# lefarov/Ape-X-DQN

Measured on AMD Instinct MI355X. Metric: learner grad-steps/sec at batch 512, 84x84x4 dueling DQN, higher is better.
Workload: dtype fp32; 1 GPU; model=dueling NatureCNN (reference DuellingDQN, conv1=64), 4x84x84, A=4, global_batch=512, seq_len=1, parallelism=dp1, batch_scope=global, per_rank_rows=512, replay_per_gpu=100000, learner=fused/hip, hip_graphs=True

## Files before the change

### apex_dqn_amd/learner/fused_learner.py

```python
from __future__ import annotations

from typing import Any, Dict, Optional

import torch

from ..config import ApexConfig
from ..models.dueling import DuellingDQN
from ..models.flat_params import (FlatLayout, flat_to_reference_state, nature_segments,
                                  reference_state_to_flat)
from ..ops.fused_ops import HipBackend, TorchBackend, split_into
from ..ops.switches import SW
from ..utils.checkpoint import (adopt_obs_scale, layout_segments, load_checkpoint, pack_flat_state,
                                save_checkpoint, unpack_flat_state, checkpoint_network)
from .dp_step import DataParallelStep, Streams
from .is_norm import IsNormMixin


def _enable_sharding(replay, comm, rt, mcap: int = 0) -> None:
    if not replay.sharded:
        seed0 = comm.broadcast_int(int(rt.seed)) if hasattr(comm, "broadcast_int") else int(rt.seed)
        replay.enable_sharding(comm.rank, comm.world_size, shard_seed=(seed0 << 20) ^ 0x5EED,
                               group=comm.group, mcap=mcap)
    replay.shard_mcap = int(mcap)
    if not rt.use_is_weights:
# ... 248 lines not shown
        if self._branched or self._dp:
            return
        nrm = (self.norm_part, 0) if self._fuse_norm else None
        self._fc_slots = ops.fc_head_wgrad(self.dH, self.y3[:B], self.G["wfc"], self.G["bfc"], self.h,
                                           self.dhead, self.G, prio, norm=nrm,
                                           **self._lo(dh_lo=self.dH_lo, x_lo=sp and self.y3_lo[:B],
                                                      Hon_lo=self.h_lo))
        if self._comm_bf16:
            cut = self.layout.offsets["wfc"]
            self.gcomm[cut:].copy_(self.g32[cut:])
        self._mark("fc_wgrad")

    def _sample(self) -> None:
        self.replay.sample(self.B, out=self.S, nxt2=self.slots[2 * self.B:])
        self._sample_ver = self.replay.version

    def _seg2(self, after_first=None) -> None:
        if self._branched:
            assert after_first is None
            return self._seg2_branched()
        B, rt, ops, G, Pb, Pl = self.B, self.rt, self.ops, self.G, self.Pb, self.Pl
        sp = self.split
        jobs = []
        ops.fc_dgrad(self.dH, self.y3[:B], Pb["wfc"], self.dY3,
                     **self._lo(dh_lo=self.dH_lo, w_lo=sp and Pl["wfc"], dx_lo=self.dY3_lo))
        if after_first is not None:
            after_first()
        ops.conv_wgrad(self.dY3, self.y2[:B], 3, 1, G["w3"], G["b3"], jobs=jobs,
                       **self._lo(dy_lo=self.dY3_lo, x_lo=sp and self.y2_lo[:B]))
        ops.conv_dgrad(self.dY3, Pb["w3"], 1, self.y2[:B], self.dY2,
                       **self._lo(dy_lo=self.dY3_lo, w_lo=sp and Pl["w3"], dx_lo=self.dY2_lo))
        ops.conv_wgrad(self.dY2, self.y1[:B], 4, 2, G["w2"], G["b2"], jobs=jobs,
                       **self._lo(dy_lo=self.dY2_lo, x_lo=sp and self.y1_lo[:B]))
        ops.conv_dgrad(self.dY2, Pb["w2"], 2, self.y1[:B], self.dY1,
                       **self._lo(dy_lo=self.dY2_lo, w_lo=sp and Pl["w2"], dx_lo=self.dY1_lo))
        jobs1 = []
        ops.conv1_wgrad_ring(self.dY1, self.replay.frames, self.slots[:B], self.frames, rt.obs_scale, G["w1"],
                             G["b1"], jobs=jobs1, **self._lo(dy_lo=self.dY1_lo))
        fuse = self._fuse_norm
        n1 = ops.finalize_grads(jobs, self.g_head_region if fuse else None,
                                dict(part=self.norm_part, slot0=self._fc_slots) if fuse else None)
        n2 = ops.finalize_grads(jobs1, None, dict(part=self.norm_part, slot0=n1) if fuse else None)
        self._npart = n2 if fuse else 0
        if self._comm_bf16:
            cut = self.layout.offsets["wfc"]
            self.gcomm[:cut].copy_(self.g32[:cut])
        self._mark("conv_backward")

    _marks = None

    def _mark(self, name: str) -> None:
        if self._marks is not None:
            ev = torch.cuda.Event(enable_timing=True)
            ev.record()
            self._marks.append((name, ev))

    def profile_step(self) -> Dict[str, float]:
        if self.device.type != "cuda":
            return {}
        start = torch.cuda.Event(enable_timing=True)
        start.record()
        self._marks = []
        try:
            if self._dp:
                self._dp_body()
            else:
                self._step_body()
        finally:
            marks, self._marks = self._marks, None
        torch.cuda.synchronize(self.device)
        out, prev = {}, start
# ... 17 lines not shown
                      **({"frag_out": self._frag_out} if (self._frag_out is not None and nxt is not None) else {}),
                      **({"segs": segs} if segs is not None else {}),
                      **({"norm_prefix": norm_prefix} if norm_prefix is not None else {}))
        if self._presample:
            self._sample_ver = self.replay.version
        self._mark("optimizer")

    def _seg2_branched(self) -> None:
        B, rt, ops, G, Pb, Pl, S = self.B, self.rt, self.ops, self.G, self.Pb, self.Pl, self.S
        sp = self.split
        main, side = torch.cuda.current_stream(self.device), self._wg_stream
        jobs = []
        prio = (self.replay, S["idx"], S["gen"], self.td_abs)
        nrm = (self.norm_part, 0) if self._fuse_norm else None

        def fc_wgrad():
            self._fc_slots = ops.fc_head_wgrad(self.dH, self.y3[:B], G["wfc"], G["bfc"], self.h, self.dhead, G,
                                               prio, norm=nrm,
                                               **self._lo(dh_lo=self.dH_lo, x_lo=sp and self.y3_lo[:B],
                                                          Hon_lo=self.h_lo))

        fc_main = SW.fc_wgrad_main == "on" or (SW.fc_wgrad_main == "auto" and sp and B >= 256)
        if not fc_main:
            ev = torch.cuda.Event()
            ev.record(main)
        ops.fc_dgrad(self.dH, self.y3[:B], Pb["wfc"], self.dY3,
                     **self._lo(dh_lo=self.dH_lo, w_lo=sp and Pl["wfc"], dx_lo=self.dY3_lo))
        if fc_main:
            fc_wgrad()
        else:
            side.wait_event(ev)
            with torch.cuda.stream(side):
                fc_wgrad()
        self._conv32_branched(main, side, jobs)
        fuse = self._fuse_norm
        jobs1 = []
        ops.conv1_wgrad_ring(self.dY1, self.replay.frames, self.slots[:B], self.frames, rt.obs_scale, G["w1"],
                             G["b1"], jobs=jobs1, **self._lo(dy_lo=self.dY1_lo))
        with torch.cuda.stream(side):
            n_side = ops.finalize_grads(jobs, self.g_head_region if fuse else None,
                                        dict(part=self.norm_part, slot0=self._fc_slots) if fuse else None)
        n_main = ops.finalize_grads(jobs1, None, dict(part=self.norm_part, slot0=n_side) if fuse else None)
        main.wait_stream(side)
        self._npart = n_main
        self._mark("conv_backward")

    def _conv2_wgrad(self, jobs) -> None:
        B, sp = self.B, self.split
        self.ops.conv_wgrad(self.dY2, self.y1[:B], 4, 2, self.G["w2"], self.G["b2"], jobs=jobs,
                            **self._lo(dy_lo=self.dY2_lo, x_lo=sp and self.y1_lo[:B]))

    def _conv3_wgrad(self, jobs) -> None:
        B, sp = self.B, self.split
        self.ops.conv_wgrad(self.dY3, self.y2[:B], 3, 1, self.G["w3"], self.G["b3"], jobs=jobs,
                            **self._lo(dy_lo=self.dY3_lo, x_lo=sp and self.y2_lo[:B]))

    def _conv32_branched(self, main, side, jobs, wgrad2: bool = True) -> None:
        B, ops, G, Pb, Pl, sp = self.B, self.ops, self.G, self.Pb, self.Pl, self.split
        ev3 = torch.cuda.Event()
        ev3.record(main)
        ops.conv_dgrad(self.dY3, Pb["w3"], 1, self.y2[:B], self.dY2,
                       **self._lo(dy_lo=self.dY3_lo, w_lo=sp and Pl["w3"], dx_lo=self.dY2_lo))
        side.wait_event(ev3)
        with torch.cuda.stream(side):
            self._conv3_wgrad(jobs)
        ev2 = torch.cuda.Event()
        ev2.record(main)
        ops.conv_dgrad(self.dY2, Pb["w2"], 2, self.y1[:B], self.dY1,
                       **self._lo(dy_lo=self.dY2_lo, w_lo=sp and Pl["w2"], dx_lo=self.dY1_lo))
        side.wait_event(ev2)
        if wgrad2:
            with torch.cuda.stream(side):
                self._conv2_wgrad(jobs)

    def _step_body(self) -> None:
        self._seg1()
        self._seg2()
        self._seg3()

    def _body(self) -> None:
        if self._dp:
            self._dp_body()
        else:
            self._step_body()
        if not self._defer_params:
            self._wait_params()

    _step_hook = None

    graph_fallback = None
    _inject_capture_failure = False

    def _graphs_enabled(self) -> bool:
        return (bool(self.rt.use_graphs) and self.device.type == "cuda" and (not self._dp or self._dp_graphs)
                and self.graph_fallback is None)

    def step(self) -> None:
        graphs = self._graphs_enabled()
        if graphs and self._graphs is None:
            self.prepare_graphs(multi=False)
            graphs = self._graphs_enabled()
        if graphs and self._presample and self._sample_ver != self.replay.version:
# ... 281 lines not shown
```

### apex_dqn_amd/ops/conv.py

```python
from __future__ import annotations

from typing import Dict, Optional, Tuple


import torch

from . import _lib
from .switches import SW


class Workspace:
    def __init__(self):
        self.bufs: Dict[Tuple, torch.Tensor] = {}

    def get(self, key, numel: int, device, dtype=torch.float32) -> torch.Tensor:
        k = (key, numel, str(device), dtype)
        t = self.bufs.get(k)
        if t is None:
            t = torch.empty(numel, dtype=dtype, device=device)
            self.bufs[k] = t
        return t

    work_queue = False

    def wq(self, key, device, overlapped: bool = True) -> int:
        mode = SW.work_queue
        on = mode == "on" or (mode != "off" and self.work_queue and overlapped)
        return self.get_zeroed(key, 1, device, dtype=torch.int64).data_ptr() if on else 0

    def get_zeroed(self, key, numel: int, device, dtype=torch.int32) -> torch.Tensor:
        k = (key, numel, str(device), dtype)
        t = self.bufs.get(k)
        if t is None:
            t = torch.zeros(numel, dtype=dtype, device=device)
            self.bufs[k] = t
        return t


_DEFAULT_WS = Workspace()

_HINTS: Dict[str, int] = {}


def set_launch_hints(tile: int = 0, order: int = 0) -> None:
    _HINTS["tile"], _HINTS["order"] = int(tile), int(order)


def _conv_desc(**kw) -> "_lib.ConvDesc":
    d = _lib.ConvDesc()
    d.x = kw.get("x")
    d.frame_slots = kw.get("frame_slots")
    d.w = kw["w"]
    d.bias = kw.get("bias")
    d.y = kw["y"]
    d.mask = kw.get("mask")
    d.N, d.H, d.W, d.Cin = kw["N"], kw.get("H", 1), kw.get("W", 1), kw["Cin"]
    d.OH, d.OW, d.Cout = kw.get("OH", 1), kw.get("OW", 1), kw["Cout"]
    d.KH, d.KW = kw.get("KH", 1), kw.get("KW", 1)
    d.stride, d.pad_h, d.pad_w = kw.get("stride", 1), kw.get("pad", 0), kw.get("pad", 0)
    d.mode, d.relu = kw["mode"], int(kw.get("relu", 0))
# ... 391 lines not shown
               "conv_wgrad")


def conv1_wgrad_ring(lib, ws: Workspace, dy: torch.Tensor, ring: torch.Tensor, slots: torch.Tensor,
                     scale: float, dw_out: torch.Tensor, db_out: torch.Tensor, grid: int = 0,
                     jobs: Optional[list] = None, dy_lo: Optional[torch.Tensor] = None) -> None:
    N, OH, OW, Co = dy.shape
    C = slots.shape[1]
    assert (OH, OW, Co) == (20, 20, 64) and slots.dtype == torch.int32 and dy.is_contiguous()
    G = grid if grid > 0 else min(N, 256)
    K = 64 * C
    slab = ws.get(("wg1img", C, G), G * 64 * K, dy.device)
    bslab = ws.get(("wg1imgb", G), G * 64, dy.device)
    zero = ws.get(("zero16",), 64, ring.device, torch.uint8)
    if not getattr(ws, "_zeroed", False):
        zero.zero_()
        ws._zeroed = True
    d = _lib.Conv1WgDesc()
    d.ring, d.slots, d.dy = ring.data_ptr(), slots.data_ptr(), dy.data_ptr()
    d.slab, d.bias_slab, d.zero16 = slab.data_ptr(), bslab.data_ptr(), zero.data_ptr()
    d.N, d.C = N, C
    d.dy_lo = _lib.ptr(dy_lo)
    d.wq = ws.wq(("c1w_wq", N, int(G)), dy.device)
    st = _lib.stream_ptr()
    _lib.check(lib.apex_conv1_wgrad_img(d, G, st), "conv1_wgrad_img")
    if jobs is not None:
        jobs.append(dict(slab=slab, bslab=bslab, out=dw_out, bout=db_out, n=64 * K, nsplit=G, nb=64, s2dC=C, Kc=K,
                         scale=float(scale)))
        return
    _lib.check(lib.apex_slab_reduce(slab.data_ptr(), G, 64 * K, float(scale), dw_out.data_ptr(), bslab.data_ptr(),
                                    64, db_out.data_ptr(), C, K, st), "slab_reduce")


def conv1_wgrad_ring_tiled(lib, ws: Workspace, dy: torch.Tensor, ring: torch.Tensor, slots: torch.Tensor,
                           scale: float, dw_out: torch.Tensor, db_out: torch.Tensor, target_rows: int = 0,
                           jobs: Optional[list] = None, dy_lo: Optional[torch.Tensor] = None) -> None:
    if target_rows <= 0:
        target_rows = 800 if dy_lo is not None else 1024
    N, OH, OW, Co = dy.shape
    C = slots.shape[1]
    Kc = C * 64
    Mred = N * OH * OW
    nsplit, rows = _splits(Mred, target_rows, _WG_TBL // C)
    slab = ws.get(("wg1", Co, Kc), nsplit * Co * Kc, dy.device)
    bslab = ws.get(("wg1b", Co), nsplit * Co, dy.device)
    d = _wg_desc(dy=dy.data_ptr(), x=ring.data_ptr(), frame_slots=slots.data_ptr(), slab=slab.data_ptr(),
                 bias_slab=bslab.data_ptr(), N=N, H=ring.shape[1], W=ring.shape[2], Cin=C, OH=OH, OW=OW,
                 KH=8, KW=8, stride=4, mode=2, Co=Co, Kc=Kc, ldd=Co, rows_per_split=rows, Mred=Mred,
                 dy_lo=_lib.ptr(dy_lo))
    if jobs is not None:
        _lib.check(lib.apex_conv_wgrad(d, None, None, nsplit, 1.0, _lib.stream_ptr()), "conv1_wgrad")
        jobs.append(dict(slab=slab, bslab=bslab, out=dw_out, bout=db_out, n=Co * Kc, nsplit=nsplit, nb=Co, s2dC=C,
                         Kc=Kc, scale=float(scale)))
        return
    _lib.check(lib.apex_conv_wgrad(d, dw_out.data_ptr(), db_out.data_ptr(), nsplit, float(scale),
                                   _lib.stream_ptr()), "conv1_wgrad")


_WG_SHAPES = ((1, 4), (2, 2), (4, 1), (1, 3), (1, 1), (1, 2), (2, 1))


def wgrad_blocks(Co: int, Kc: int, sp: int = 0) -> int:
    kt, ct = Kc // 64, Co // 64
    best, bc = (1, 1), None
    for i, (c, n) in enumerate(_WG_SHAPES):
        if kt % n or ct % c:
# ... 106 lines not shown
```

### apex_dqn_amd/ops/conv_sigs.py

```python
from __future__ import annotations

import ctypes

c_p = ctypes.c_void_p
c_i = ctypes.c_int
c_i64 = ctypes.c_int64
c_f = ctypes.c_float


class Conv2ImgDesc(ctypes.Structure):
    _fields_ = [("x", c_p), ("w", c_p), ("w2", c_p), ("bias", c_p), ("bias2", c_p), ("y", c_p),
                ("N", c_i), ("img_switch", c_i), ("x_lo", c_p), ("w_lo", c_p), ("w2_lo", c_p), ("y_lo", c_p),
                ("wfrag", c_p), ("wfrag_ready", c_i)]


class Conv12Desc(ctypes.Structure):
    _fields_ = [("ring", c_p), ("slots", c_p), ("w1", c_p), ("w1b", c_p), ("b1", c_p), ("b1b", c_p),
                ("w2", c_p), ("w2_lo", c_p), ("w2b", c_p), ("w2b_lo", c_p), ("wfrag", c_p), ("pack_sets", c_i),
                ("b2", c_p), ("b2b", c_p), ("y1", c_p), ("y1_lo", c_p), ("y2", c_p), ("y2_lo", c_p),
                ("w1frag", c_p), ("scratch", c_p), ("N", c_i), ("C", c_i), ("img_switch", c_i), ("copy_n", c_i),
                ("in_scale", ctypes.c_float), ("probe", c_p), ("wq", c_p), ("bf16", c_i), ("probe_split", c_i),
                ("w3", c_p), ("w3_lo", c_p), ("w3b", c_p), ("w3b_lo", c_p), ("b3", c_p), ("b3b", c_p),
                ("y3", c_p), ("y3_lo", c_p), ("w3frag", c_p)]


class Conv2DgradImgDesc(ctypes.Structure):
    _fields_ = [("dy", c_p), ("w", c_p), ("mask", c_p), ("dx", c_p), ("N", c_i), ("dy_lo", c_p), ("w_lo", c_p),
                ("dx_lo", c_p), ("wfrag", c_p), ("wfrag_ready", c_i), ("wq", c_p), ("cls_split", c_i)]


class C2dPackJob(ctypes.Structure):
    _fields_ = [("w", c_p), ("w_lo", c_p), ("out", c_p)]


class Conv3DgradImgDesc(ctypes.Structure):
    _fields_ = [("dy", c_p), ("w", c_p), ("mask", c_p), ("dx", c_p), ("N", c_i)]


def declare(lib: ctypes.CDLL) -> None:
    from ._lib import ConvDesc, WgradDesc
    sigs = {
        "apex_conv2_img_fwd": ([Conv2ImgDesc, c_i, c_p], c_i),
        "apex_conv12_fused_fwd": ([Conv12Desc, c_i, c_p], c_i),
        "apex_conv12_pack": ([Conv12Desc, c_p], c_i),
        "apex_conv2_dgrad_img": ([Conv2DgradImgDesc, c_i, c_p], c_i),
        "apex_conv3_dgrad_img": ([Conv3DgradImgDesc, c_i, c_p], c_i),
        "apex_conv_fwd": ([ConvDesc, c_p], c_i),
        "apex_fc_gemm128": ([ConvDesc, c_p, c_i64, c_i, c_i, c_i, C2dPackJob, c_p], c_i),
        "apex_conv_wgrad": ([WgradDesc, c_p, c_p, c_i, c_f, c_p], c_i),
        "apex_pack_dgrad_weights": ([c_p, c_p, c_p, c_p, c_p, c_p, c_p], c_i),
    }
    for name, (args, res) in sigs.items():
        fn = getattr(lib, name, None)
        if fn is None:
            continue
        fn.argtypes = args
        fn.restype = res
```

### apex_dqn_amd/ops/fused_ops.py

```python
from __future__ import annotations

import ctypes
from typing import Dict, Optional

import torch

from . import _lib
from . import conv as C
from . import reference as R
from .switches import SW


def join(hi: torch.Tensor, lo: Optional[torch.Tensor]) -> torch.Tensor:
    return hi.float() if lo is None else hi.float() + lo.float()


def split_into(v: torch.Tensor, hi: torch.Tensor, lo: Optional[torch.Tensor]) -> None:
    hi.copy_(v.reshape(hi.shape))
    if lo is not None:
        lo.copy_((v.reshape(hi.shape).float() - hi.float()))


class TorchBackend:
    name = "torch"
# ... 171 lines not shown

    def fc_wgrad_split(self, dh, x, dw_out, db_out, jobs, split_rows: int, jnorm, dh_lo=None, x_lo=None,
                       cpb: int = -1) -> int:
        return self.fc_wgrad(dh, x, dw_out, db_out, norm=(jnorm, 0), dh_lo=dh_lo, x_lo=x_lo)

    def fc_head_wgrad(self, dh, x, dw_out, db_out, Hon, dhead, g_head, prio, norm=None, dh_lo=None, x_lo=None,
                      Hon_lo=None) -> int:
        self.head_wgrad(Hon, dhead, g_head, prio=prio, Hon_lo=Hon_lo)
        return self.fc_wgrad(dh, x, dw_out, db_out, norm=norm, dh_lo=dh_lo, x_lo=x_lo) or 0

    def finalize_grads(self, jobs, norm_range=None, norm=None) -> int:
        return 0

    def conv_dgrad(self, dy, w, stride, x_src, dx_out, dy_lo=None, w_lo=None, dx_lo=None):
        if dy_lo is not None:
            dx = R.conv_dgrad(join(dy, dy_lo), join(w, w_lo), tuple(x_src.shape), stride, x_src, torch.float32)
            split_into(dx, dx_out, dx_lo)
            return
        dx_out.copy_(R.conv_dgrad(dy, w, tuple(x_src.shape), stride, x_src, self.dtype))

    def conv_wgrad(self, dy, x, k, stride, dw_out, db_out, jobs=None, dy_lo=None, x_lo=None):
        dw, db = R.conv_wgrad(join(dy, dy_lo), join(x, x_lo), k, stride)
        dw_out.copy_(dw)
        db_out.copy_(db)

    def conv1_wgrad(self, dy, frames, scale, dw_out, db_out, dy_lo=None):
        dw, db = R.conv1_wgrad(join(dy, dy_lo), frames, scale)
        dw_out.copy_(dw)
        db_out.copy_(db)

    def conv1_wgrad_ring(self, dy, ring, slots, frames_buf, scale, dw_out, db_out, jobs=None, dy_lo=None):
        self.conv1_wgrad(dy, frames_buf[:slots.shape[0]], scale, dw_out, db_out, dy_lo=dy_lo)

    def optimizer(self, p32, g32, v, m, pbf, lr, alpha, eps, clip, centered, partials, norm_out, norm_total=None,
                  sample=None, pb_lo=None, wnorm=None, frag_out=None, segs=None, norm_prefix=None):
        self._optimizer(p32, g32, v, m, pbf, lr, alpha, eps, clip, centered, norm_out, pb_lo, wnorm, norm_total,
                        segs, norm_prefix)
        if sample is not None:
            rp, B, out, nxt2 = sample
            rp.sample(B, out=out, nxt2=nxt2)

    def _optimizer(self, p32, g32, v, m, pbf, lr, alpha, eps, clip, centered, norm_out, pb_lo=None, wnorm=None,
                   norm_total=None, segs=None, norm_prefix=None):
        sc = torch.ones((), dtype=torch.float32, device=g32.device)
        if wnorm is not None:
            st, n, stride = wnorm
            mx = st.reshape(-1)[0:n * stride:stride].max().float()
            sc = torch.where(mx > 0, 1.0 / mx.clamp_min(1e-30), sc)
        if norm_total is not None:
            part, npart = norm_total if isinstance(norm_total, tuple) else (norm_total, 1)
            sq = part[:npart].double().sum()
            if norm_prefix is not None:
                sq = sq + norm_prefix.double().pow(2).sum()
        else:
            assert segs is None, "a sharded update needs the clip norm's partials (norm_total)"
            sq = g32.double().pow(2).sum()
        norm = sq.sqrt().float() * sc
        coef = torch.clamp(clip / (norm + 1e-6), max=1.0) if clip > 0 else torch.ones_like(norm)
        for o, n in (segs if segs is not None else [(0, p32.numel())]):
            r = slice(o, o + n)
            g = g32[r] * (coef * sc)
            vr, mr, pr = v[r], m[r], p32[r]
            vr.mul_(alpha).add_((1 - alpha) * g * g)
            if centered:
                mr.mul_(alpha).add_((1 - alpha) * g)
                var = vr - mr * mr
# ... 139 lines not shown
                return r
        return super().fc_head_wgrad(dh, x, dw_out, db_out, Hon, dhead, g_head, prio, norm, dh_lo, x_lo, Hon_lo)

    def finalize_grads(self, jobs, norm_range=None, norm=None) -> int:
        if not jobs and norm is None:
            return 0
        if norm is None:
            C.finalize_grads(self.lib, jobs)
            return 0
        return norm["slot0"] + C.finalize_grads(self.lib, jobs, norm_range, norm["part"], norm["slot0"],
                                                norm.get("total"))

    def conv_dgrad(self, dy, w, stride, x_src, dx_out, dy_lo=None, w_lo=None, dx_lo=None):
        if not self.native_conv:
            return super().conv_dgrad(dy, w, stride, x_src, dx_out, dy_lo, w_lo, dx_lo)
        if stride == 1:
            C.conv3_dgrad(self.lib, dy, w, x_src, dx_out, dy_lo=dy_lo, w_lo=w_lo, out_lo=dx_lo)
        else:
            key = (w.data_ptr(), _lib.ptr(w_lo))
            packed = getattr(self, "_c2d_packed", None) == key
            self._c2d_packed = None
            C.conv2_dgrad(self.lib, dy, w, x_src, dx_out, dy_lo=dy_lo, w_lo=w_lo, out_lo=dx_lo, ws=self.ws,
                          packed=packed)

    def conv_wgrad(self, dy, x, k, stride, dw_out, db_out, jobs=None, dy_lo=None, x_lo=None):
        if not self.native_conv:
            return super().conv_wgrad(dy, x, k, stride, dw_out, db_out, dy_lo=dy_lo, x_lo=x_lo)
        C.conv_wgrad(self.lib, self.ws, dy, x, k, stride, dw_out, db_out, jobs=jobs, dy_lo=dy_lo, x_lo=x_lo)

    def conv1_wgrad_ring(self, dy, ring, slots, frames_buf, scale, dw_out, db_out, jobs=None, dy_lo=None):
        if not self.native_conv:
            return super().conv1_wgrad_ring(dy, ring, slots, frames_buf, scale, dw_out, db_out, dy_lo=dy_lo)
        C.conv1_wgrad_ring(self.lib, self.ws, dy, ring, slots, scale, dw_out, db_out, jobs=jobs, dy_lo=dy_lo)

    @staticmethod
    def _hp(P):
        h = _lib.HeadParams()
        h.wv, h.bv, h.wa, h.ba = (P["wv"].data_ptr(), P["bv"].data_ptr(), P["wa"].data_ptr(),
                                  P["ba"].data_ptr())
        return h

    def head(self, Hon, Htg, Pon, Ptg, act, rew, gam, isw, huber, kappa, grad_scale, td_abs, loss, dH,
             dhead, q_out=None, zero=None, lo=None, isn=None):
        B = act.shape[0]
        A = Pon["wa"].shape[0]
        args = (Hon.data_ptr(), Htg.data_ptr(), self._hp(Pon), self._hp(Ptg), act.data_ptr(), rew.data_ptr(),
                gam.data_ptr(), _lib.ptr(isw), B, A, int(huber), float(kappa), float(grad_scale),
                td_abs.data_ptr(), loss.data_ptr(), _lib.ptr(q_out), dH.data_ptr(), dhead.data_ptr(),
                _lib.ptr(zero), 0 if zero is None else zero.numel(), Pon["wv"].numel())
        hl = _lib.head_lo(*(lo if lo is not None else (None, None, None)))
        hp, pk = _lib.HeadPart(), _lib.C2dPack()
        fp = getattr(self, "_fc_part", None)
        if fp is not None:
            self._fc_part = None
            assert fp["out"].data_ptr() == Hon.data_ptr() and fp["two_b"] == 2 * B
            hp.part, hp.zstride, hp.nz = fp["part"].data_ptr(), int(fp["zstride"]), int(fp["nz"])
            hp.bias_on, hp.bias_tg, hp.two_b = fp["b"].data_ptr(), fp["b2"].data_ptr(), int(fp["two_b"])
            hp.hon, hp.hon_lo = Hon.data_ptr(), _lib.ptr(None if lo is None else lo[0])
            if fp["c2d"] is not None:
                pk.w, pk.w_lo = fp["c2d"][0].data_ptr(), _lib.ptr(fp["c2d"][1])
                pk.out = C.c2d_wfrag_buffer(self.ws, Hon.device).data_ptr()
                self._c2d_packed = (fp["c2d"][0].data_ptr(), _lib.ptr(fp["c2d"][1]))
        isn_s = _lib.IsNorm()
        if isn is not None:
            isn_s.wscale, isn_s.out = _lib.ptr(isn[0]), _lib.ptr(isn[1])
            isn_s.valid_count = _lib.ptr(isn[2]) if len(isn) > 2 else None
# ... 117 lines not shown
```

### apex_dqn_amd/ops/switches.py

```python
from __future__ import annotations

import dataclasses
import os
from dataclasses import dataclass
from typing import Any, Dict


@dataclass
class Switches:
    conv2_img: bool = True
    c2f_pack: bool = True
    conv12_fused: bool = True
    conv123_max_images: int = 1 << 20
    conv12_bf16: bool = True
    conv3_dgrad_img: bool = True
    conv2_dgrad_img: bool = True
    conv2_dgrad_cls_max: int = 256
    opt_frags: bool = True
    fc_epi_in_head: bool = True
    bwd_branches: bool = True
    actor_fc_ksplit: int = 4
    fc_wgrad_main: str = "auto"
    fc_ksplit_max: int = 0
    work_queue: str = "auto"
    wg_rows3: int = 0
    wg_rows2: int = 0
    impala_wg_target: int = 512
    impala_slab_cap: int = 8 << 20
    resblock_r16: int = 14
    impala_pool_wgrad: bool = True
    isplit_bands: str = ""
    dp_fc_shard_branch: bool = False
    dp_branch_one_wait: bool = True
    dp_fc_split_rows: int = -1
    dp_norm_split: bool = True

    @classmethod
    def from_env(cls, spec: str = None) -> "Switches":
        sw = cls()
        spec = os.environ.get("APEX_SWITCHES", "") if spec is None else spec
        for item in spec.split(","):
            item = item.strip()
            if not item:
                continue
            if "=" not in item:
                raise ValueError(f"APEX_SWITCHES item must be name=value, got {item!r}")
            k, v = item.split("=", 1)
            f = {f.name: f for f in dataclasses.fields(cls)}.get(k)
            if f is None:
                raise ValueError(f"unknown kernel switch {k!r}")
# ... 20 lines not shown
```

Baseline: 2705 grad-steps/s (batch 512).

## Fuse conv2 dgrad with conv1 wgrad into one persistent per-image HIP kernel

Adds a persistent kernel that computes conv2's input gradient per image in LDS, applies the ReLU mask, and immediately uses that tile together with DMA-loaded ring frames to accumulate conv1 weight and bias gradients into per-block slabs. The intermediate dY1 no longer needs to be written to and re-read from global memory, and one kernel launch is removed from the backward pass. The kernel uses large LDS and 512 threads with one block per CU, and pipelines the next image's frame and dy loads behind the current image's MFMA work. It is enabled by default on the branched and unbranched backward paths when batch exceeds the class-split threshold, C=4, and the work queue is off. A fallback to the previous two-kernel path is kept.

```diff
diff --git a/apex_dqn_amd/csrc/conv21_bwd_fused.hip b/apex_dqn_amd/csrc/conv21_bwd_fused.hip
--- /dev/null
+++ b/apex_dqn_amd/csrc/conv21_bwd_fused.hip
@@ -0,0 +1,299 @@
+#include "mfma_common.h"
+#include "conv2_wfrag.h"
+
+typedef float f32x16 __attribute__((ext_vector_type(16)));
+
+struct Conv21BwdDesc {
+  const bf16_t* dy;
+  const bf16_t* dy_lo;
+  const bf16_t* w;
+  const bf16_t* w_lo;
+  const bf16_t* mask;
+  uint4* wfrag;
+  int wfrag_ready;
+  const uint8_t* ring;
+  const int32_t* slots;
+  const uint8_t* zero16;
+  float* slab;
+  float* bias_slab;
+  bf16_t* dx;
+  bf16_t* dx_lo;
+  unsigned long long* wq;
+  int N, C;
+};
+
+#define F21_THREADS 512
+#define F21_PLANE 7168
+#define F21_IMG (8 * F21_PLANE)
+#define F21_DYPL (256 * 128)
+#define F21_S2PL (144 * 128)
+#define F21_NCHUNK (4 * 441)
+#define F21_NDMA 28
+#define F21_NDY2 11
+
+__device__ __forceinline__ int f21_c2d_off(int slot, int c) { return (slot << 7) + ((c ^ ((slot >> 1) & 7)) << 4); }
+
+__global__ void __launch_bounds__(256) pack_c2d_wfrag21_kernel(const bf16_t* __restrict__ w,
+                                                               const bf16_t* __restrict__ w_lo,
+                                                               uint32_t* __restrict__ out) {
+  pack_c2d_wfrag_word(blockIdx.x * 256 + threadIdx.x, w, w_lo, out);
+}
+
+__global__ void __launch_bounds__(F21_THREADS, 1) conv21_bwd_fused_kernel(Conv21BwdDesc d) {
+  __shared__ __attribute__((aligned(16))) uint8_t smem[F21_IMG + 2 * F21_DYPL + 2 * F21_S2PL];
+  uint8_t* Pl = smem;
+  uint8_t* Dy = Pl + F21_IMG;
+  uint8_t* S2 = Dy + 2 * F21_DYPL;
+  uint8_t* Sg = S2;
+  const int tid = threadIdx.x, lane = tid & 63;
+  const int wv = __builtin_amdgcn_readfirstlane(tid >> 6);
+  const int cls = wv >> 1, nh = wv & 1, p = cls >> 1, q = cls & 1;
+  const int rr = lane & 31, kg = lane >> 5;
+  const int g = lane >> 4, qq = (lane >> 2) & 3, pcol = lane & 3;
+  const int wc = wv & 1, wk = wv >> 1;
+  const int G = gridDim.x;
+
+  bf16x8 wh[16], wl[16];
+  {
+    const uint4* __restrict__ wf = d.wfrag + ((cls * 2 + nh) * 16) * 64 + lane;
+#pragma unroll
+    for (int s = 0; s < 16; ++s) {
+      wh[s] = __builtin_bit_cast(bf16x8, wf[s * 64]);
+      wl[s] = __builtin_bit_cast(bf16x8, wf[C2D_FRAGS + s * 64]);
+    }
+  }
+  int xoff[4];
+#pragma unroll
+  for (int j = 0; j < 4; ++j)
+    xoff[j] = (2 * j + (pcol >> 1)) * F21_PLANE + (((wk >> 1) * 21 + (wk & 1)) << 4) + ((pcol & 1) << 3);
+
+  auto issue_frames = [&](int img) {
+    int sl[4];
+    sload_slots<4>(d.slots + img * 4, sl);
+    int ln = lane;
+    asm volatile("" : "+v"(ln));
+#pragma unroll
+    for (int i = 0; i < 4; ++i) {
+      const int k = wv * 4 + i;
+      if (k < F21_NDMA) {
+        const int j = 64 * k + ln;
+        const uint8_t* src = d.zero16;
+        if (j < F21_NCHUNK) {
+          const int c = j / 441, blk = j - c * 441;
+          int slot = sl[0];
+#pragma unroll
+          for (int cc = 1; cc < 4; ++cc)
+            if (c == cc) slot = sl[cc];
+          src = d.ring + (int64_t)slot * 7056 + (blk << 4);
+        }
+        const uint32_t off = (uint32_t)(uintptr_t)(__attribute__((address_space(3))) uint8_t*)(Sg + k * 1024);
+        dma16(src, __builtin_amdgcn_readfirstlane(off));
+      }
+    }
+  };
+  auto convert_frames = [&]() {
+    for (int j = tid; j < F21_NCHUNK; j += F21_THREADS) {
+      const uint4 v = *reinterpret_cast<const uint4*>(Sg + j * 16);
+      const int c = j / 441, blk = j - c * 441;
+      *reinterpret_cast<uint4*>(Pl + (2 * c) * F21_PLANE + blk * 16) = u8x8_to_bf16x8(v.x, v.y);
+      *reinterpret_cast<uint4*>(Pl + (2 * c + 1) * F21_PLANE + blk * 16) = u8x8_to_bf16x8(v.z, v.w);
+    }
+  };
+  auto issue_dy2 = [&](int img) {
+    int ln = lane;
+    asm volatile("" : "+v"(ln));
+#pragma unroll
+    for (int i = 0; i < 3; ++i) {
+      const int k = wv + 8 * i;
+      if (k < 2 * F21_NDY2) {
+        const int pln = k / F21_NDY2, kk = k - pln * F21_NDY2, j = 64 * kk + ln;
+        const uint8_t* src = d.zero16;
+        if (j < 81 * 8) src = reinterpret_cast<const uint8_t*>((pln ? d.dy_lo : d.dy) + (int64_t)img * 81 * 64) + j * 16;
+        const uint32_t off =
+            (uint32_t)(uintptr_t)(__attribute__((address_space(3))) uint8_t*)(Dy + pln * F21_DYPL + 160 * 128 + kk * 1024);
+        dma16(src, __builtin_amdgcn_readfirstlane(off));
+      }
+    }
+  };
+  auto store_dy2 = [&]() {
+    for (int k = tid; k < 2 * 144 * 8; k += F21_THREADS) {
+      const int pl = k >= 144 * 8 ? 1 : 0, kk = k - pl * 144 * 8;
+      const int slot = kk >> 3, c = (kk & 7) ^ ((slot >> 1) & 7);
+      const int row = slot / 11, col = slot - row * 11;
+      uint4 v = make_uint4(0, 0, 0, 0);
+      if (row >= 1 && row <= 9 && col >= 1 && col <= 9)
+        v = *reinterpret_cast<const uint4*>(Dy + pl * F21_DYPL + 160 * 128 + (((row - 1) * 9 + col - 1) * 8 + c) * 16);
+      *reinterpret_cast<uint4*>(S2 + k * 16) = v;
+    }
+  };
+
+  f32x4 acc[2][4], accb[2];
+#pragma unroll
+  for (int i = 0; i < 2; ++i) {
+    accb[i] = (f32x4){0.f, 0.f, 0.f, 0.f};
+#pragma unroll
+    for (int j = 0; j < 4; ++j) acc[i][j] = (f32x4){0.f, 0.f, 0.f, 0.f};
+  }
+  const bf16x8 ones = __builtin_bit_cast(bf16x8, make_uint4(0x3f803f80u, 0x3f803f80u, 0x3f803f80u, 0x3f803f80u));
+
+  auto wg_steps = [&](int ks0, int ks1, int lk0) {
+#pragma unroll 1
+    for (int ks = ks0; ks < ks1; ++ks) {
+      const int p0 = min(32 * ks + 8 * g + qq, 399), p1 = min(32 * ks + 8 * g + qq + 4, 399);
+      const int oh0 = p0 / 20, oh1 = p1 / 20;
+      const int b0 = ((oh0 * 21 + p0 - 20 * oh0) << 4), b1 = ((oh1 * 21 + p1 - 20 * oh1) << 4);
+      const int lk = ks - ks0 + lk0;
+      bf16x8 a[2], al[2], b[4];
+#pragma unroll
+      for (int i = 0; i < 2; ++i) {
+        a[i] = tr_frag8(Dy, lk, 16 * (2 * wc + i), lane);
+        al[i] = tr_frag8(Dy + F21_DYPL, lk, 16 * (2 * wc + i), lane);
+      }
+#pragma unroll
+      for (int j = 0; j < 4; ++j) {
+        const lds_s16x4* pa = (const lds_s16x4*)(Pl + b0 + xoff[j]);
+        const lds_s16x4* pb = (const lds_s16x4*)(Pl + b1 + xoff[j]);
+        s16x4 lo = __builtin_amdgcn_ds_read_tr16_b64_v4i16(const_cast<lds_s16x4*>(pa));
+        s16x4 hi = __builtin_amdgcn_ds_read_tr16_b64_v4i16(const_cast<lds_s16x4*>(pb));
+        typedef short s16x8 __attribute__((ext_vector_type(8)));
+        b[j] = __builtin_bit_cast(bf16x8, (s16x8){lo[0], lo[1], lo[2], lo[3], hi[0], hi[1], hi[2], hi[3]});
+      }
+#pragma unroll
+      for (int i = 0; i < 2; ++i)
+#pragma unroll
+        for (int j = 0; j < 4; ++j) {
+          acc[i][j] = __builtin_amdgcn_mfma_f32_16x16x32_bf16(b[j], al[i], acc[i][j], 0, 0, 0);
+          acc[i][j] = __builtin_amdgcn_mfma_f32_16x16x32_bf16(b[j], a[i], acc[i][j], 0, 0, 0);
+        }
+      if (wk == 0) {
+#pragma unroll
+        for (int i = 0; i < 2; ++i) {
+          accb[i] = __builtin_amdgcn_mfma_f32_16x16x32_bf16(ones, al[i], accb[i], 0, 0, 0);
+          accb[i] = __builtin_amdgcn_mfma_f32_16x16x32_bf16(ones, a[i], accb[i], 0, 0, 0);
+        }
+      }
+    }
+  };
+
+  int img = blockIdx.x;
+  if (img < d.N) {
+    issue_dy2(img);
+    issue_frames(img);
+  }
+  for (; img < d.N; img += G) {
+    asm volatile("s_waitcnt vmcnt(0)" ::: "memory");
+    __syncthreads();
+    convert_frames();
+    __syncthreads();
+    store_dy2();
+    __syncthreads();
+    const uint2* __restrict__ mbase = reinterpret_cast<const uint2*>(d.mask + (int64_t)img * 400 * 64);
+#pragma unroll
+    for (int tp = 0; tp < 2; ++tp) {
+#pragma unroll
+      for (int t = 0; t < 2; ++t) {
+        int rq = rr;
+        asm volatile("" : "+v"(rq));
+        const int rt = (tp == 0 ? 0 : 60) + t * 32 + rq;
+        const bool valid = rt < (tp == 0 ? 60 : 100);
+        const int r = min(rt, 99);
+        const int pi = r / 10, pj = r - pi * 10;
+        const int px = (2 * pi + p) * 20 + 2 * pj + q;
+        const int rho = px < 256 ? px : px - 256;
+        uint2 mv[4];
+#pragma unroll
+        for (int g4 = 0; g4 < 4; ++g4) mv[g4] = mbase[px * 16 + nh * 8 + 2 * g4 + kg];
+        f32x16 dacc;
+#pragma unroll
+        for (int j = 0; j < 16; ++j) dacc[j] = 0.f;
+        bf16x8 xf[2][2];
+#define F21_LDX(s_, dst_)                                                                    \
+        {                                                                                    \
+          const int off_ = f21_c2d_off((pi - (((s_) >> 3) & 1) + 1) * 11 + (pj - (((s_) >> 2) & 1) + 1), \
+                                       (((s_) & 3) << 1) | kg);                              \
+          dst_[0] = __builtin_bit_cast(bf16x8, *reinterpret_cast<const uint4*>(S2 + off_)); \
+          dst_[1] = __builtin_bit_cast(bf16x8, *reinterpret_cast<const uint4*>(S2 + F21_S2PL + off_)); \
+        }
+        F21_LDX(0, xf[0])
+#pragma unroll
+        for (int s = 0; s < 16; ++s) {
+          if (s + 1 < 16) F21_LDX(s + 1, xf[(s + 1) & 1])
+          __builtin_amdgcn_sched_barrier(0);
+          dacc = __builtin_amdgcn_mfma_f32_32x32x16_bf16(wl[s], xf[s & 1][0], dacc, 0, 0, 0);
+          dacc = __builtin_amdgcn_mfma_f32_32x32x16_bf16(wh[s], xf[s & 1][1], dacc, 0, 0, 0);
+          dacc = __builtin_amdgcn_mfma_f32_32x32x16_bf16(wh[s], xf[s & 1][0], dacc, 0, 0, 0);
+          __builtin_amdgcn_sched_barrier(0);
+        }
+#undef F21_LDX
+        if (valid) {
+          const int sw = (((rho >> 1) & 1) | (((rho >> 3) & 1) << 1)) << 1;
+#pragma unroll
+          for (int g4 = 0; g4 < 4; ++g4) {
+            uint32_t h01, l01, h23, l23;
+            split_pk_bf16(dacc[4 * g4], dacc[4 * g4 + 1], h01, l01);
+            split_pk_bf16(dacc[4 * g4 + 2], dacc[4 * g4 + 3], h23, l23);
+            const uint2 m = mv[g4];
+            const uint2 vh = make_uint2(mask_bf16x2(h01, m.x), mask_bf16x2(h23, m.y));
+            const uint2 vl = make_uint2(mask_bf16x2(l01, m.x), mask_bf16x2(l23, m.y));
+            const int o = (rho << 7) + (((nh * 4 + g4) ^ sw) << 4) + kg * 8;
+            *reinterpret_cast<uint2*>(Dy + o) = vh;
+            *reinterpret_cast<uint2*>(Dy + F21_DYPL + o) = vl;
+            if (d.dx != nullptr) {
+              const int64_t go = ((int64_t)img * 400 + px) * 64 + nh * 32 + 8 * g4 + 4 * kg;
+              *reinterpret_cast<uint2*>(d.dx + go) = vh;
+              *reinterpret_cast<uint2*>(d.dx_lo + go) = vl;
+            }
+          }
+        }
+      }
+      if (tp == 1 && tid < 256)
+        *reinterpret_cast<uint4*>(Dy + (tid >> 7) * F21_DYPL + 144 * 128 + (tid & 127) * 16) = make_uint4(0, 0, 0, 0);
+      __syncthreads();
+      if (tp == 0) {
+        wg_steps(0, 7, 0);
+        __syncthreads();
+      } else {
+        if (img + G < d.N) issue_frames(img + G);
+        wg_steps(7, 8, 7);
+        if (img + G < d.N) {
+          __syncthreads();
+          issue_dy2(img + G);
+        }
+        wg_steps(8, 13, 0);
+      }
+    }
+  }
+
+  float* slab = d.slab + (int64_t)blockIdx.x * 64 * 256;
+  const int pl = lane & 15;
+#pragma unroll
+  for (int i = 0; i < 2; ++i)
+#pragma unroll
+    for (int j = 0; j < 4; ++j) {
+      const int co = 16 * (2 * wc + i) + pl;
+      *reinterpret_cast<f32x4*>(slab + (int64_t)co * 256 + 16 * (4 * wk + j) + 4 * g) = acc[i][j];
+    }
+  if (wk == 0 && g == 0) {
+#pragma unroll
+    for (int i = 0; i < 2; ++i) d.bias_slab[(int64_t)blockIdx.x * 64 + 16 * (2 * wc + i) + pl] = accb[i][0];
+  }
+}
+
+APEX_EXPORT int apex_conv21_bwd_fused(Conv21BwdDesc d, int grid, hipStream_t st) {
+  if (d.N <= 0 || grid <= 0 || d.C != 4 || d.wq != nullptr) return (int)hipErrorInvalidValue;
+  if (d.dy == nullptr || d.dy_lo == nullptr || d.mask == nullptr || d.wfrag == nullptr || d.ring == nullptr ||
+      d.slots == nullptr || d.zero16 == nullptr || d.slab == nullptr || d.bias_slab == nullptr)
+    return (int)hipErrorInvalidValue;
+  if (((uintptr_t)d.dy | (uintptr_t)d.dy_lo | (uintptr_t)d.mask | (uintptr_t)d.wfrag | (uintptr_t)d.ring |
+       (uintptr_t)d.slots | (uintptr_t)d.zero16 | (uintptr_t)d.slab) & 15)
+    return (int)hipErrorInvalidValue;
+  if ((uintptr_t)d.bias_slab & 3) return (int)hipErrorInvalidValue;
+  if ((d.dx == nullptr) != (d.dx_lo == nullptr) || (((uintptr_t)d.dx | (uintptr_t)d.dx_lo) & 15))
+    return (int)hipErrorInvalidValue;
+  if (!d.wfrag_ready) {
+    if (d.w == nullptr || d.w_lo == nullptr) return (int)hipErrorInvalidValue;
+    pack_c2d_wfrag21_kernel<<<C2D_PACK_THREADS / 256, 256, 0, st>>>(d.w, d.w_lo, reinterpret_cast<uint32_t*>(d.wfrag));
+  }
+  conv21_bwd_fused_kernel<<<grid, F21_THREADS, 0, st>>>(d);
+  APEX_CHECK_LAUNCH();
+}
diff --git a/apex_dqn_amd/learner/fused_learner.py b/apex_dqn_amd/learner/fused_learner.py
--- a/apex_dqn_amd/learner/fused_learner.py
+++ b/apex_dqn_amd/learner/fused_learner.py
@@ -304,11 +304,10 @@
                        **self._lo(dy_lo=self.dY3_lo, w_lo=sp and Pl["w3"], dx_lo=self.dY2_lo))
         ops.conv_wgrad(self.dY2, self.y1[:B], 4, 2, G["w2"], G["b2"], jobs=jobs,
                        **self._lo(dy_lo=self.dY2_lo, x_lo=sp and self.y1_lo[:B]))
-        ops.conv_dgrad(self.dY2, Pb["w2"], 2, self.y1[:B], self.dY1,
-                       **self._lo(dy_lo=self.dY2_lo, w_lo=sp and Pl["w2"], dx_lo=self.dY1_lo))
         jobs1 = []
-        ops.conv1_wgrad_ring(self.dY1, self.replay.frames, self.slots[:B], self.frames, rt.obs_scale, G["w1"],
-                             G["b1"], jobs=jobs1, **self._lo(dy_lo=self.dY1_lo))
+        ops.conv2_dgrad_conv1_wgrad(self.dY2, Pb["w2"], self.y1[:B], self.dY1, self.replay.frames, self.slots[:B],
+                                    self.frames, rt.obs_scale, G["w1"], G["b1"], jobs=jobs1,
+                                    **self._lo(dy2_lo=self.dY2_lo, w2_lo=sp and Pl["w2"], dy1_lo=self.dY1_lo))
         fuse = self._fuse_norm
         n1 = ops.finalize_grads(jobs, self.g_head_region if fuse else None,
                                 dict(part=self.norm_part, slot0=self._fc_slots) if fuse else None)
@@ -392,11 +391,13 @@
             side.wait_event(ev)
             with torch.cuda.stream(side):
                 fc_wgrad()
-        self._conv32_branched(main, side, jobs)
+        jobs1 = []
+        fuse21 = ops.conv21_fused_ok(self.dY2, self.slots[:B], **self._lo(dy2_lo=self.dY2_lo, w2_lo=sp and Pl["w2"]))
+        self._conv32_branched(main, side, jobs, jobs1=jobs1 if fuse21 else None)
+        if not fuse21:
+            ops.conv1_wgrad_ring(self.dY1, self.replay.frames, self.slots[:B], self.frames, rt.obs_scale, G["w1"],
+                                 G["b1"], jobs=jobs1, **self._lo(dy_lo=self.dY1_lo))
         fuse = self._fuse_norm
-        jobs1 = []
-        ops.conv1_wgrad_ring(self.dY1, self.replay.frames, self.slots[:B], self.frames, rt.obs_scale, G["w1"],
-                             G["b1"], jobs=jobs1, **self._lo(dy_lo=self.dY1_lo))
         with torch.cuda.stream(side):
             n_side = ops.finalize_grads(jobs, self.g_head_region if fuse else None,
                                         dict(part=self.norm_part, slot0=self._fc_slots) if fuse else None)
@@ -415,8 +416,8 @@
         self.ops.conv_wgrad(self.dY3, self.y2[:B], 3, 1, self.G["w3"], self.G["b3"], jobs=jobs,
                             **self._lo(dy_lo=self.dY3_lo, x_lo=sp and self.y2_lo[:B]))
 
-    def _conv32_branched(self, main, side, jobs, wgrad2: bool = True) -> None:
-        B, ops, G, Pb, Pl, sp = self.B, self.ops, self.G, self.Pb, self.Pl, self.split
+    def _conv32_branched(self, main, side, jobs, wgrad2: bool = True, jobs1=None) -> None:
+        B, ops, G, Pb, Pl, sp, rt = self.B, self.ops, self.G, self.Pb, self.Pl, self.split, self.rt
         ev3 = torch.cuda.Event()
         ev3.record(main)
         ops.conv_dgrad(self.dY3, Pb["w3"], 1, self.y2[:B], self.dY2,
@@ -426,8 +427,13 @@
             self._conv3_wgrad(jobs)
         ev2 = torch.cuda.Event()
         ev2.record(main)
-        ops.conv_dgrad(self.dY2, Pb["w2"], 2, self.y1[:B], self.dY1,
-                       **self._lo(dy_lo=self.dY2_lo, w_lo=sp and Pl["w2"], dx_lo=self.dY1_lo))
+        if jobs1 is None:
+            ops.conv_dgrad(self.dY2, Pb["w2"], 2, self.y1[:B], self.dY1,
+                           **self._lo(dy_lo=self.dY2_lo, w_lo=sp and Pl["w2"], dx_lo=self.dY1_lo))
+        else:
+            ops.conv2_dgrad_conv1_wgrad(self.dY2, Pb["w2"], self.y1[:B], self.dY1, self.replay.frames,
+                                        self.slots[:B], self.frames, rt.obs_scale, G["w1"], G["b1"], jobs=jobs1,
+                                        **self._lo(dy2_lo=self.dY2_lo, w2_lo=sp and Pl["w2"], dy1_lo=self.dY1_lo))
         side.wait_event(ev2)
         if wgrad2:
             with torch.cuda.stream(side):
diff --git a/apex_dqn_amd/ops/conv.py b/apex_dqn_amd/ops/conv.py
--- a/apex_dqn_amd/ops/conv.py
+++ b/apex_dqn_amd/ops/conv.py
@@ -23,9 +23,12 @@
 
     work_queue = False
 
+    def wq_on(self, overlapped: bool = True) -> bool:
+        mode = SW.work_queue
+        return mode == "on" or (mode != "off" and self.work_queue and overlapped)
+
     def wq(self, key, device, overlapped: bool = True) -> int:
-        mode = SW.work_queue
-        on = mode == "on" or (mode != "off" and self.work_queue and overlapped)
+        on = self.wq_on(overlapped)
         return self.get_zeroed(key, 1, device, dtype=torch.int64).data_ptr() if on else 0
 
     def get_zeroed(self, key, numel: int, device, dtype=torch.int32) -> torch.Tensor:
@@ -483,6 +486,49 @@
                                     64, db_out.data_ptr(), C, K, st), "slab_reduce")
 
 
+def conv2_dgrad_conv1_wgrad_fused(lib, ws: Workspace, dy: torch.Tensor, dy_lo: torch.Tensor, w2: torch.Tensor,
+                                  w_lo: torch.Tensor, mask: torch.Tensor, ring: torch.Tensor, slots: torch.Tensor,
+                                  scale: float, dw_out: torch.Tensor, db_out: torch.Tensor, grid: int = 0,
+                                  jobs: Optional[list] = None, packed: bool = False,
+                                  dx: Optional[torch.Tensor] = None, dx_lo: Optional[torch.Tensor] = None,
+                                  wq: int = 0) -> None:
+    from .conv_sigs import Conv21BwdDesc
+    N = dy.shape[0]
+    C = slots.shape[1]
+    assert tuple(dy.shape) == (N, 9, 9, 64) and tuple(mask.shape) == (N, 20, 20, 64)
+    assert tuple(w2.shape) == (64, 4, 4, 64) and slots.dtype == torch.int32 and slots.shape[0] == N
+    assert dy.is_contiguous() and mask.is_contiguous() and w2.is_contiguous() and slots.is_contiguous()
+    for t in (dy_lo, w_lo):
+        assert t is not None and t.is_contiguous() and t.dtype == torch.bfloat16
+    for t in (dx, dx_lo):
+        assert t is None or (tuple(t.shape) == (N, 20, 20, 64) and t.is_contiguous() and t.dtype == torch.bfloat16)
+    G = grid if grid > 0 else min(N, 256)
+    K = 64 * C
+    slab = ws.get(("wg1img", C, G), G * 64 * K, dy.device)
+    bslab = ws.get(("wg1imgb", G), G * 64, dy.device)
+    zero = ws.get(("zero16",), 64, ring.device, torch.uint8)
+    if not getattr(ws, "_zeroed", False):
+        zero.zero_()
+        ws._zeroed = True
+    d = Conv21BwdDesc()
+    d.dy, d.dy_lo, d.w, d.w_lo, d.mask = dy.data_ptr(), dy_lo.data_ptr(), w2.data_ptr(), w_lo.data_ptr(), mask.data_ptr()
+    d.wfrag = c2d_wfrag_buffer(ws, dy.device).data_ptr()
+    d.wfrag_ready = int(packed)
+    d.ring, d.slots, d.zero16 = ring.data_ptr(), slots.data_ptr(), zero.data_ptr()
+    d.slab, d.bias_slab = slab.data_ptr(), bslab.data_ptr()
+    d.dx, d.dx_lo = _lib.ptr(dx), _lib.ptr(dx_lo)
+    d.wq = wq or None
+    d.N, d.C = N, C
+    st = _lib.stream_ptr()
+    _lib.check(lib.apex_conv21_bwd_fused(d, G, st), "conv21_bwd_fused")
+    if jobs is not None:
+        jobs.append(dict(slab=slab, bslab=bslab, out=dw_out, bout=db_out, n=64 * K, nsplit=G, nb=64, s2dC=C, Kc=K,
+                         scale=float(scale)))
+        return
+    _lib.check(lib.apex_slab_reduce(slab.data_ptr(), G, 64 * K, float(scale), dw_out.data_ptr(), bslab.data_ptr(),
+                                    64, db_out.data_ptr(), C, K, st), "slab_reduce")
+
+
 def conv1_wgrad_ring_tiled(lib, ws: Workspace, dy: torch.Tensor, ring: torch.Tensor, slots: torch.Tensor,
                            scale: float, dw_out: torch.Tensor, db_out: torch.Tensor, target_rows: int = 0,
                            jobs: Optional[list] = None, dy_lo: Optional[torch.Tensor] = None) -> None:
diff --git a/apex_dqn_amd/ops/conv_sigs.py b/apex_dqn_amd/ops/conv_sigs.py
--- a/apex_dqn_amd/ops/conv_sigs.py
+++ b/apex_dqn_amd/ops/conv_sigs.py
@@ -29,6 +29,12 @@
                 ("dx_lo", c_p), ("wfrag", c_p), ("wfrag_ready", c_i), ("wq", c_p), ("cls_split", c_i)]
 
 
+class Conv21BwdDesc(ctypes.Structure):
+    _fields_ = [("dy", c_p), ("dy_lo", c_p), ("w", c_p), ("w_lo", c_p), ("mask", c_p), ("wfrag", c_p),
+                ("wfrag_ready", c_i), ("ring", c_p), ("slots", c_p), ("zero16", c_p), ("slab", c_p),
+                ("bias_slab", c_p), ("dx", c_p), ("dx_lo", c_p), ("wq", c_p), ("N", c_i), ("C", c_i)]
+
+
 class C2dPackJob(ctypes.Structure):
     _fields_ = [("w", c_p), ("w_lo", c_p), ("out", c_p)]
 
@@ -45,6 +51,7 @@
         "apex_conv12_pack": ([Conv12Desc, c_p], c_i),
         "apex_conv2_dgrad_img": ([Conv2DgradImgDesc, c_i, c_p], c_i),
         "apex_conv3_dgrad_img": ([Conv3DgradImgDesc, c_i, c_p], c_i),
+        "apex_conv21_bwd_fused": ([Conv21BwdDesc, c_i, c_p], c_i),
         "apex_conv_fwd": ([ConvDesc, c_p], c_i),
         "apex_fc_gemm128": ([ConvDesc, c_p, c_i64, c_i, c_i, c_i, C2dPackJob, c_p], c_i),
         "apex_conv_wgrad": ([WgradDesc, c_p, c_p, c_i, c_f, c_p], c_i),
diff --git a/apex_dqn_amd/ops/fused_ops.py b/apex_dqn_amd/ops/fused_ops.py
--- a/apex_dqn_amd/ops/fused_ops.py
+++ b/apex_dqn_amd/ops/fused_ops.py
@@ -227,6 +227,14 @@
     def conv1_wgrad_ring(self, dy, ring, slots, frames_buf, scale, dw_out, db_out, jobs=None, dy_lo=None):
         self.conv1_wgrad(dy, frames_buf[:slots.shape[0]], scale, dw_out, db_out, dy_lo=dy_lo)
 
+    def conv21_fused_ok(self, dy2, slots, dy2_lo=None, w2_lo=None) -> bool:
+        return False
+
+    def conv2_dgrad_conv1_wgrad(self, dy2, w2, y1, dy1, ring, slots, frames_buf, scale, dw_out, db_out, jobs=None,
+                                dy2_lo=None, w2_lo=None, dy1_lo=None):
+        self.conv_dgrad(dy2, w2, 2, y1, dy1, dy_lo=dy2_lo, w_lo=w2_lo, dx_lo=dy1_lo)
+        self.conv1_wgrad_ring(dy1, ring, slots, frames_buf, scale, dw_out, db_out, jobs=jobs, dy_lo=dy1_lo)
+
     def optimizer(self, p32, g32, v, m, pbf, lr, alpha, eps, clip, centered, partials, norm_out, norm_total=None,
                   sample=None, pb_lo=None, wnorm=None, frag_out=None, segs=None, norm_prefix=None):
         self._optimizer(p32, g32, v, m, pbf, lr, alpha, eps, clip, centered, norm_out, pb_lo, wnorm, norm_total,
@@ -432,6 +440,22 @@
         if not self.native_conv:
             return super().conv1_wgrad_ring(dy, ring, slots, frames_buf, scale, dw_out, db_out, dy_lo=dy_lo)
         C.conv1_wgrad_ring(self.lib, self.ws, dy, ring, slots, scale, dw_out, db_out, jobs=jobs, dy_lo=dy_lo)
+
+    def conv21_fused_ok(self, dy2, slots, dy2_lo=None, w2_lo=None) -> bool:
+        return bool(self.native_conv and SW.conv21_bwd_fused and SW.conv2_dgrad_img and dy2_lo is not None
+                    and w2_lo is not None and slots.shape[1] == 4 and dy2.shape[0] > SW.conv2_dgrad_cls_max
+                    and hasattr(self.lib, "apex_conv21_bwd_fused") and not self.ws.wq_on())
+
+    def conv2_dgrad_conv1_wgrad(self, dy2, w2, y1, dy1, ring, slots, frames_buf, scale, dw_out, db_out, jobs=None,
+                                dy2_lo=None, w2_lo=None, dy1_lo=None):
+        if self.conv21_fused_ok(dy2, slots, dy2_lo, w2_lo):
+            packed = getattr(self, "_c2d_packed", None) == (w2.data_ptr(), _lib.ptr(w2_lo))
+            self._c2d_packed = None
+            C.conv2_dgrad_conv1_wgrad_fused(self.lib, self.ws, dy2, dy2_lo, w2, w2_lo, y1, ring, slots, scale,
+                                            dw_out, db_out, jobs=jobs, packed=packed)
+            return
+        super().conv2_dgrad_conv1_wgrad(dy2, w2, y1, dy1, ring, slots, frames_buf, scale, dw_out, db_out, jobs=jobs,
+                                        dy2_lo=dy2_lo, w2_lo=w2_lo, dy1_lo=dy1_lo)
 
     @staticmethod
     def _hp(P):
diff --git a/apex_dqn_amd/ops/switches.py b/apex_dqn_amd/ops/switches.py
--- a/apex_dqn_amd/ops/switches.py
+++ b/apex_dqn_amd/ops/switches.py
@@ -16,6 +16,7 @@
     conv3_dgrad_img: bool = True
     conv2_dgrad_img: bool = True
     conv2_dgrad_cls_max: int = 256
+    conv21_bwd_fused: bool = True
     opt_frags: bool = True
     fc_epi_in_head: bool = True
     bwd_branches: bool = True
```

New measurement: 2853 grad-steps/s (batch 512), median of 6. +5.5%, better.
